# TianmingQiu/BNN_KFAC

Measured on AMD Instinct MI355X. Metric: images/sec for full KFAC factor pass + factor inversion, MNIST MLP, 1/2/4/8 GPUs, higher is better.
Workload: dtype f32; 1 GPU; C2: MLP 784-128-10 KFAC factor pass over 60000 images/rank (batch 4096/rank, global batch 4096) + invert(0.04000000000000001, 200); global_batch=4096, images_per_rank=60000, parallelism=dp1

## Files before the change

bnn_kfac_amd/_native.py:

```python
from __future__ import annotations

import atexit
import ctypes
import os
import threading

import torch

_HERE = os.path.dirname(os.path.abspath(__file__))
LIB_PATH = os.environ.get("BNN_KFAC_AMD_LIB", os.path.join(_HERE, "libkfac_hip.so"))

KFAC_OK, KFAC_EINVAL, KFAC_ELAUNCH, KFAC_EWORKSPACE = 0, -1, -2, -3
ROWMAJOR, CHANNEL, PATCH = 0, 1, 2
OUT_INV_CHOL, OUT_INVERSE = 0, 1
TRI_SYMMETRIC, TRI_LOWER = 0, 1
(PROF_FACTOR_TILES, PROF_FACTOR_REDUCE, PROF_INVERT, PROF_QUAD_TILES, PROF_FACTOR_SYRK3,
 PROF_FACTOR_X3, PROF_FACTOR_CONV, PROF_FACTOR_CHANNEL_SMALL, PROF_SYEV, PROF_FACTOR_CONV_X3,
 PROF_FACTOR_CONV_X3S, PROF_FACTOR_CONV_X3F, PROF_FACTOR_CHANNEL_X3) = range(13)
PROF_FACTOR_KERNELS = {PROF_FACTOR_TILES: "kfac_factor_tiles", PROF_FACTOR_SYRK3: "kfac_factor_syrk3",
                       PROF_FACTOR_X3: "kfac_factor_tiles_x3", PROF_FACTOR_CONV: "kfac_factor_conv",
                       PROF_FACTOR_CHANNEL_SMALL: "kfac_factor_channel_small",
                       PROF_FACTOR_CONV_X3: "kfac_factor_conv_x3", PROF_FACTOR_CONV_X3S: "kfac_factor_conv_x3s",
                       PROF_FACTOR_CONV_X3F: "kfac_factor_conv_x3f", PROF_FACTOR_CHANNEL_X3: "kfac_factor_channel_x3"}

# ... 83 lines not shown
                ("ld_diag", c_i64), ("nA", c_i32), ("nG", c_i32), ("accumulate", c_i32),
                ("scale", c_f32)]


class GramJob(ctypes.Structure):
    _fields_ = [("UA", c_vp), ("ldA", c_i64), ("UG", c_vp), ("ldG", c_i64), ("c", c_vp),
                ("sigma", c_vp), ("out", c_vp), ("ldo", c_i64), ("nA", c_i32), ("nG", c_i32),
                ("la", c_i32), ("lg", c_i32)]


class TriJob(ctypes.Structure):
    _fields_ = [("F", c_vp), ("ldF", c_i64), ("n", c_i32), ("reserved", c_i32), ("offset", c_i64)]


SIGNATURES = {
    "kfac_factor_workspace_bytes": (ctypes.c_size_t, [ctypes.POINTER(FactorJob), ctypes.c_int]),
    "kfac_factor_update": (ctypes.c_int, [ctypes.POINTER(FactorJob), ctypes.c_int, c_vp,
                                          ctypes.c_size_t, c_vp]),
    "kfac_factor_accum_plan": (ctypes.c_int, [ctypes.POINTER(FactorJob), ctypes.c_int,
                                              ctypes.POINTER(c_i32), ctypes.POINTER(ctypes.c_size_t)]),
    "kfac_factor_route": (ctypes.c_int, [ctypes.POINTER(FactorJob), ctypes.c_int, ctypes.POINTER(c_i32)]),
    "kfac_factor_flush": (ctypes.c_int, [ctypes.POINTER(FactorJob), ctypes.c_int, c_vp]),
    "kfac_x3_unit_table": (ctypes.c_int, [ctypes.c_int, ctypes.POINTER(c_i32), ctypes.c_int]),
    "kfac_syrk_linear": (ctypes.c_int, [c_vp, c_i64, c_i64, c_i64, ctypes.c_int, c_f32, c_f32,
                                        c_vp, c_i64, c_vp, ctypes.c_size_t, c_vp]),
    "kfac_syrk_conv": (ctypes.c_int, [c_vp, c_i64] + [ctypes.c_int] * 10 + [c_f32, c_f32, c_vp,
                                                                            c_i64, c_vp,
                                                                            ctypes.c_size_t, c_vp]),
    "kfac_syrk_convgrad": (ctypes.c_int, [c_vp, c_i64, ctypes.c_int, c_i64, c_f32, c_f32, c_vp,
                                          c_i64, c_vp, ctypes.c_size_t, c_vp]),
    "kfac_invert_workspace_bytes": (ctypes.c_size_t, [ctypes.POINTER(InvertJob), ctypes.c_int]),
    "kfac_invert": (ctypes.c_int, [ctypes.POINTER(InvertJob), ctypes.c_int, c_vp,
                                   ctypes.c_size_t, c_vp, c_vp]),
    "kfac_invert_ex": (ctypes.c_int, [ctypes.POINTER(InvertJob), ctypes.c_int, c_vp,
                                      ctypes.c_size_t, c_vp, c_vp, c_vp]),
    "kfac_damped_inv_chol": (ctypes.c_int, [c_vp, ctypes.c_int, c_i64, c_f64, c_f64, c_vp, c_i64,
                                            c_vp, ctypes.c_size_t, c_vp, c_vp]),
    "kfac_eig_workspace_bytes": (ctypes.c_size_t, [ctypes.POINTER(EigJob), ctypes.c_int]),
    "kfac_syev": (ctypes.c_int, [ctypes.POINTER(EigJob), ctypes.c_int, c_vp, ctypes.c_size_t,
                                 c_vp, c_vp]),
    "kfac_quadform_workspace_bytes": (ctypes.c_size_t, [ctypes.POINTER(QuadJob), ctypes.c_int,
                                                        c_i64]),
    "kfac_kron_quadform": (ctypes.c_int, [ctypes.POINTER(QuadJob), ctypes.c_int, c_i64,
                                          ctypes.c_int, c_vp, c_vp, ctypes.c_size_t, c_vp]),
    "kfac_kron_cov_workspace_bytes": (ctypes.c_size_t, [ctypes.POINTER(CovJob), ctypes.c_int, c_i64,
                                                        ctypes.c_int]),
# ... 663 lines not shown
```

bnn_kfac_amd/csrc/capi.hip:

```cpp
#include "kfac_common.h"

extern "C" const char* kfac_strerror(int status) {
  switch (status) {
    case KFAC_OK: return "ok";
    case KFAC_EINVAL: return "invalid argument";
    case KFAC_ELAUNCH: return "HIP kernel launch failed";
    case KFAC_EWORKSPACE: return "workspace too small";
    default: return "unknown kfac status";
  }
}

extern "C" const char* kfac_version(void) { return "bnn_kfac_amd 0.1.0 gfx950"; }

#include <stdlib.h>
#include <string.h>

#include <algorithm>
#include <atomic>

#include "knobs.h"

namespace kfac {
namespace {
int env_int(const char* name, int dflt) {
// ... 121 lines not shown
  int64_t cnt = 0;
  for (const Rec& r : g_done) {
    if (r.id != id) continue;
    if (hipEventSynchronize(r.stop) != hipSuccess) return KFAC_ELAUNCH;
    float ms = 0.f;
    if (hipEventElapsedTime(&ms, r.start, r.stop) != hipSuccess) return KFAC_ELAUNCH;
    tot += ms;
    wk += r.work;
    by += r.bytes;
    ++cnt;
  }
  if (total_ms) *total_ms = tot;
  if (launches) *launches = cnt;
  if (work) *work = wk;
  if (bytes) *bytes = by;
  return KFAC_OK;
}

extern "C" int kfac_profile_read(int id, double* total_ms, int64_t* launches) {
  return kfac_profile_read_work(id, total_ms, launches, nullptr, nullptr);
}

int kfac_release_graphs();

extern "C" int kfac_release(void) {
  int rc = kfac_release_graphs();
  std::lock_guard<std::mutex> lk(g_mu);
  g_on = false;
  for (const Rec& r : g_open) {
    (void)hipEventDestroy(r.start);
    (void)hipEventDestroy(r.stop);
  }
  for (const Rec& r : g_done) {
    if (hipEventSynchronize(r.stop) != hipSuccess) rc = KFAC_ELAUNCH;
    (void)hipEventDestroy(r.start);
    (void)hipEventDestroy(r.stop);
  }
  for (hipEvent_t e : g_pool) (void)hipEventDestroy(e);
  g_open.clear();
  g_done.clear();
  g_pool.clear();
  return rc;
}

extern "C" int kfac_event_create(void** ev) {
  if (!ev) return KFAC_EINVAL;
  return hipEventCreateWithFlags(reinterpret_cast<hipEvent_t*>(ev), hipEventDisableTiming) == hipSuccess
             ? KFAC_OK
             : KFAC_ELAUNCH;
// ... 35 lines not shown
```

bnn_kfac_amd/csrc/factor.hip:

```cpp
#include <algorithm>
#include <utility>
#include <vector>

#include "factor_common.h"

namespace kfac {

struct Plan {
  int tiles, splits;
  int units;
  int tasks;
  int64_t chunk;
  size_t slab_bytes;
};

static int factor_n(const kfac_factor_job& j) { return j.x.cols + (j.x.has_ones ? 1 : 0); }

static int64_t job_sps(const kfac_factor_job& j) { return std::max<int64_t>(1, cdiv(j.x.rows, BK)); }
static int job_nseg(const kfac_factor_job& j) { return j.nseg > 1 ? j.nseg : 1; }
static bool job_ragged(const kfac_factor_job& j) {
  return j.nseg > 1 && j.x.last_rows > 0 && j.x.last_rows < j.x.rows;
}
static int64_t job_stages(const kfac_factor_job& j) {
  if (job_ragged(j)) return job_sps(j) * (j.nseg - 1) + std::max<int64_t>(1, cdiv(j.x.last_rows, BK));
  return job_sps(j) * job_nseg(j);
}
static int64_t job_krows(const kfac_factor_job& j) {
  if (job_ragged(j)) return j.x.rows * (j.nseg - 1) + j.x.last_rows;
  return j.x.rows * job_nseg(j);
}
static double job_operand_bytes(const kfac_factor_job& j) {
  const double rows = (double)job_krows(j);
  if (j.x.layout == KFAC_PATCH)
    return rows / (double)std::max<int64_t>(1, j.x.L) * (double)j.x.C * j.x.H * j.x.W * sizeof(float);
  return rows * j.x.cols * sizeof(float);
}
// ... 97 lines not shown
    const uintptr_t* bases = reinterpret_cast<const uintptr_t*>(j.seg_ptrs);
    for (int64_t s = 0; s < nseg; ++s)
      if (bases[s] % 16 != 0) return false;
  }
  if (!conv_fp32_geom(o, g)) return false;
  r.family = o.layout != KFAC_CHANNEL ? KFAC_PROF_FACTOR_CONV
             : channel_small(g)       ? KFAC_PROF_FACTOR_CHANNEL_SMALL
             : channel_x3_geom(o, g)  ? KFAC_PROF_FACTOR_CHANNEL_X3 : KFAC_PROF_FACTOR_CONV;
  return true;
}

static Route route_group(const kfac_factor_job* jobs, int njobs) {
  Route r{};
  r.family = KFAC_PROF_FACTOR_TILES;
  if (syrk3_group(jobs, njobs))
    r.family = KFAC_PROF_FACTOR_SYRK3;
  else if (tiles_x3_group(jobs, njobs))
    r.family = KFAC_PROF_FACTOR_X3;
  else if (njobs == 1)
    conv_geom(jobs[0], r);
  return r;
}

static void plan_jobs(const kfac_factor_job* jobs, int njobs, const Route& route, Plan* plans) {
  const Family& fam = family_of(route);
  const bool s3 = route.family == KFAC_PROF_FACTOR_SYRK3, x3 = route.family == KFAC_PROF_FACTOR_X3;
  const int64_t slots = (int64_t)fam.wgs * 256;
  constexpr int64_t MIN_CHUNK = 8, OVERHEAD = 4;
  int64_t max_steps = 1;
  for (int i = 0; i < njobs; ++i) max_steps = std::max(max_steps, job_stages(jobs[i]));
  int64_t units[MAXJ];
  for (int i = 0; i < njobs; ++i) {
    const int n = factor_n(jobs[i]);
    const int64_t t = cdiv(n, TILE);
    units[i] = s3 ? syrk3_units(n) : x3 ? x3_units(n) : fam.images ? route.cg.units : t * (t + 1) / 2;
  }
  auto thin = [&](int i) {
    const int n = factor_n(jobs[i]);
    return x3 && n > TILE && (n - 1) % TILE < 32;
  };
  auto job_tasks = [&](int i, int64_t splits) { return units[i] * splits; };
  auto job_splits = [&](int i, int64_t c) { return cdiv(job_stages(jobs[i]), c); };
  auto tasks_at = [&](int64_t c) {
    int64_t n = 0;
    for (int i = 0; i < njobs; ++i)
      n += job_tasks(i, job_splits(i, c));
    return n;
  };
  int64_t best_c = std::max(MIN_CHUNK, max_steps), best_cost = -1;
  bool any_thin = false;
  for (int i = 0; i < njobs; ++i) any_thin |= thin(i);
  const int64_t max_rounds = any_thin ? 1 : (s3 ? 16 : 4);
  for (int64_t r = 1; r <= max_rounds; ++r) {
    int64_t lo = MIN_CHUNK, hi = std::max(MIN_CHUNK, max_steps);
    if (tasks_at(hi) > r * slots) continue;
    while (lo < hi) {
      const int64_t mid = (lo + hi) / 2;
      if (tasks_at(mid) <= r * slots) hi = mid; else lo = mid + 1;
    }
    const int64_t cost = (lo + OVERHEAD) * r;
    if (best_cost < 0 || cost < best_cost) { best_cost = cost; best_c = lo; }
  }
  for (int i = 0; i < njobs; ++i) {
    const int t = (int)cdiv(factor_n(jobs[i]), TILE);
    Plan& p = plans[i];
    p.tiles = t * (t + 1) / 2;
    p.units = (int)units[i];
    const int64_t steps = job_stages(jobs[i]);
    if (jobs[i].acc) {
      p.splits = jobs[i].acc_splits;
      p.chunk = cdiv(steps, (int64_t)p.splits);
      p.slab_bytes = 0;
      p.tasks = (int)job_tasks(i, p.splits);
      continue;
    }
    p.splits = (int)job_splits(i, best_c);
    if (fam.images) {
      const ConvGeom& cg = route.cg;
      const bool halve = route.family == KFAC_PROF_FACTOR_CHANNEL_SMALL && cg.B <= 8 * slots;
      int k = (int)std::max<int64_t>(1, cdiv((int64_t)cg.units * cg.B, halve ? slots / 2 : slots));
      if (knobs().conv_k > 0) k = knobs().conv_k;
      k = std::min(k, cg.B);
      p.splits = (int)cdiv(cg.B, k);
    }
    p.chunk = cdiv(steps, (int64_t)p.splits);
    p.slab_bytes = align_up((size_t)p.tiles * p.splits * TILE * TILE * sizeof(float), 256);
    p.tasks = (int)job_tasks(i, p.splits);
  }
}

static size_t accum_bytes(int n, int splits) {
// ... 34 lines not shown
  d.rdelta = 0;
  if (job_ragged(jb)) {
    d.rdelta = (int)(jb.x.rows - jb.x.last_rows);
    d.rstage = (int64_t)d.sps * (jb.nseg - 1);
    d.rw = (float)((double)jb.x.rows / (double)jb.x.last_rows);
    d.rinv = (float)((double)jb.x.last_rows / (double)jb.x.rows);
  }
}

struct GroupLaunch {
  FactorArgs args, red;
  int tasks, rtiles;
};

static int prepare_group(const kfac_factor_job* jobs, int njobs, const Route& route, char* ws,
                         size_t ws_bytes, GroupLaunch& g) {
  Plan plans[MAXJ];
  plan_jobs(jobs, njobs, route, plans);
  FactorArgs& args = g.args;
  FactorArgs& red = g.red;
  args = FactorArgs{};
  red = FactorArgs{};
  args.njobs = njobs;
  args.split_major = 1;
  int tasks = 0, rtiles = 0, nsegs = 0;
  size_t off = 0;
  for (int i = 0; i < njobs; ++i) {
    const kfac_factor_job& jb = jobs[i];
    FactorJobDev& d = args.job[i];
    fill_dev(d, jb);
    d.glds = job_glds(jb);
    d.x3units = route.family == KFAC_PROF_FACTOR_X3 ? plans[i].units : 0;
    d.splits = plans[i].splits;
    d.sstride = jb.acc && jb.acc_stride > 0 ? jb.acc_stride : d.splits;
    d.chunk = plans[i].chunk;
    if (d.nseg > 1) {
      const float* const* bases = reinterpret_cast<const float* const*>(jb.seg_ptrs);
      d.seg_off = nsegs;
      for (int s = 0; s < d.nseg; ++s) args.segs[nsegs++] = bases[s];
    }
    if (jb.acc) {
      d.slab = jb.acc;
    } else {
      d.slab = reinterpret_cast<float*>(ws + off);
      off += plans[i].slab_bytes;
      FactorJobDev& e = red.job[red.njobs];
      e = d;
      e.tile_begin = rtiles;
      rtiles += plans[i].tiles;
      red.tile_end[red.njobs++] = rtiles;
    }
    d.task_begin = tasks;
    tasks += plans[i].tasks;
    args.task_end[i] = tasks;
  }
  g.tasks = tasks;
  g.rtiles = rtiles;
  return off > ws_bytes ? KFAC_EWORKSPACE : KFAC_OK;
}

static int factor_group(const kfac_factor_job* jobs, int njobs, const Route& route, char* ws,
                        size_t ws_bytes, hipStream_t stream) {
  GroupLaunch g;
  const int rc = prepare_group(jobs, njobs, route, ws, ws_bytes, g);
  if (rc != KFAC_OK) return rc;
  if (g.tasks == 0) return KFAC_OK;
  {
    double work = 0.0, bytes = 0.0;
    if (prof_on())
      for (int i = 0; i < njobs; ++i) {
// ... 65 lines not shown
    if (j.acc && (j.acc_splits <= 0 || j.acc_splits > (1 << 20))) return KFAC_EINVAL;
    if (j.acc && j.acc_stride != 0 && (j.acc_stride < j.acc_splits || j.acc_stride > (1 << 20)))
      return KFAC_EINVAL;
    if (j.nseg < 0 || (j.nseg > 1 && !j.seg_ptrs) || job_sps(j) > (1 << 30))
      return KFAC_EINVAL;
    if (j.x.last_rows < 0 || j.x.last_rows > j.x.rows ||
        (job_ragged(j) && j.x.layout != KFAC_ROWMAJOR))
      return KFAC_EINVAL;
  }
  return KFAC_OK;
}

extern "C" int kfac_factor_accum_plan(const kfac_factor_job* jobs, int njobs, int32_t* splits,
                                      size_t* bytes) {
  if (validate(jobs, njobs) != KFAC_OK || (njobs > 0 && (!splits || !bytes))) return KFAC_EINVAL;
  std::vector<kfac_factor_job> sorted;
  std::vector<int> order;
  std::vector<std::pair<int, int>> groups;
  launch_groups(jobs, njobs, sorted, order, groups);
  for (auto& j : sorted) j.acc = nullptr;
  for (const auto& g : groups) {
    Plan plans[MAXJ];
    const kfac_factor_job* gj = sorted.data() + g.first;
    plan_jobs(gj, g.second, route_group(gj, g.second), plans);
    for (int k = 0; k < g.second; ++k) {
      const int i = order[g.first + k];
      splits[i] = plans[k].splits;
      bytes[i] = accum_bytes(factor_n(jobs[i]), plans[k].splits);
    }
  }
  return KFAC_OK;
}

extern "C" int kfac_factor_route(const kfac_factor_job* jobs, int njobs, int32_t* family) {
  if (validate(jobs, njobs) != KFAC_OK || (njobs > 0 && !family)) return KFAC_EINVAL;
  std::vector<kfac_factor_job> sorted;
  std::vector<int> order;
  std::vector<std::pair<int, int>> groups;
  launch_groups(jobs, njobs, sorted, order, groups);
  for (const auto& g : groups) {
    const int fam = route_group(sorted.data() + g.first, g.second).family;
    for (int k = 0; k < g.second; ++k) family[order[g.first + k]] = fam;
  }
  return KFAC_OK;
}

static int update_group(const kfac_factor_job* gj, int n, void* workspace, size_t workspace_bytes,
// ... 189 lines not shown
```

bnn_kfac_amd/csrc/factor_common.h:

```cpp
#pragma once

#include <cstddef>

#include "kfac_common.h"

namespace kfac {

constexpr int MAXJ = 16;
constexpr int KSEG = 64;

struct FactorJobDev {
  OpDev x;
  float alpha, beta;
  float* F;
  int64_t ldF;
  float* slab;
  int seg_off;
  int64_t chunk;
  int64_t nst;
  int sps, nseg;
  int n, t, splits;
  int task_begin;
  int glds;
  int tile_begin;
  int accum;
// ... 54 lines not shown
    if (i >= nb) break;
#pragma unroll
    for (int v = 0; v < 16; ++v) *at(i, v) = upd ? fmaf(J.sbeta, old[i][v], a * acc[i][v]) : a * acc[i][v];
  }
}

__device__ __forceinline__ const float* seg_base(const FactorJobDev& J, const float* const* segs,
                                                 int seg) {
  return J.seg_off >= 0 ? segs[J.seg_off + seg] : J.x.ptr;
}

__device__ __forceinline__ int64_t seg_rows(const FactorJobDev& J, int seg) {
  return J.x.rows - (int64_t)(seg == J.nseg - 1) * J.rdelta;
}

template <int NA>
__device__ __forceinline__ void scale_acc(floatx16 (&acc)[NA], float f) {
#pragma unroll
  for (int a = 0; a < NA; ++a)
#pragma unroll
    for (int v = 0; v < 16; ++v) acc[a][v] *= f;
}

struct StageCursor {
  int seg;
  int64_t k;
  __device__ __forceinline__ void init(const FactorJobDev& J, int64_t s) {
    seg = (int)(s / J.sps);
    k = (s - (int64_t)seg * J.sps) * BK;
  }
  __device__ __forceinline__ void next(int64_t rows) {
    k += BK;
    if (k >= rows) { k = 0; ++seg; }
  }
};

template <int NW = 4>
__device__ __forceinline__ void store_narrow(const FactorJobDev& J, float* out, floatx16& acc,
                                             float* lds) {
  const int lane = threadIdx.x & 63, wave = threadIdx.x >> 6;
  __syncthreads();
  if (wave > 0) {
#pragma unroll
    for (int v = 0; v < 16; ++v) lds[((wave - 1) * 16 + v) * 64 + lane] = acc[v];
  }
  __syncthreads();
  if (wave != 0) return;
#pragma unroll
  for (int w = 0; w < NW - 1; ++w)
#pragma unroll
    for (int v = 0; v < 16; ++v) acc[v] += lds[(w * 16 + v) * 64 + lane];
  put_partial(J, acc, [&](int v) { return &out[acc_row(v, lane) * TILE + (lane & 31)]; });
}

template <int NW = 4>
__device__ __forceinline__ void narrow_direct_load(const FactorJobDev& J, const float* base, int64_t k0,
                                                   int64_t rows, float (&v)[BK / (2 * NW)]) {
  const int lane = threadIdx.x & 63, wave = threadIdx.x >> 6, rr = lane & 31, h = lane >> 5;
#pragma unroll
  for (int s2 = 0; s2 < BK / (2 * NW); ++s2) {
    const int64_t k = k0 + 2 * (wave * (BK / (2 * NW)) + s2) + h;
    v[s2] = k < rows ? (rr < J.x.cols ? base[k * J.x.ld + rr] : (rr == J.x.ones ? 1.f : 0.f)) : 0.f;
  }
}

template <int NW = 4>
__device__ __forceinline__ void factor_task_narrow_direct(const FactorJobDev& J, const float* const* segs,
                                                          int local, float* lds) {
  constexpr int NV = BK / (2 * NW);
  const int split = local;
  const int64_t s0 = (int64_t)split * J.chunk;
  const int64_t s1 = min(J.nst, s0 + J.chunk);
  floatx16 acc[1];
#pragma unroll
  for (int v = 0; v < 16; ++v) acc[0][v] = 0.f;
  if (s1 > s0) {
    StageCursor c;
    c.init(J, s0);
    const float* base = seg_base(J, segs, c.seg);
    float cur[NV], nxt[NV];
    narrow_direct_load<NW>(J, base, c.k, seg_rows(J, c.seg), cur);
    for (int64_t s = s0; s < s1; ++s) {
      const int seg = c.seg;
      c.next(J.x.rows);
      if (s + 1 < s1) {
        if (c.seg != seg) base = seg_base(J, segs, c.seg);
        narrow_direct_load<NW>(J, base, c.k, seg_rows(J, c.seg), nxt);
      }
      if (s == J.rstage && s > s0) scale_acc(acc, J.rinv);
#pragma unroll
      for (int s2 = 0; s2 < NV; ++s2)
        acc[0] = __builtin_amdgcn_mfma_f32_32x32x2f32(cur[s2], cur[s2], acc[0], 0, 0, 0);
#pragma unroll
      for (int s2 = 0; s2 < NV; ++s2) cur[s2] = nxt[s2];
    }
    if (J.rstage >= 0 && s1 > J.rstage) scale_acc(acc, J.rw);
  }
  store_narrow<NW>(J, J.slab + (size_t)split * TILE * TILE, acc[0], lds);
}

constexpr int CONV_SRC_MAX = 2048;

typedef float floatx4 __attribute__((ext_vector_type(4)));

enum ConvMode {
  CONV_BLOCKS = 0,
  CONV_N16 = 2,
  CONV_N32 = 3,
};

struct ConvGeom {
  int mode;
  int n;
  int KR;
  int B;
  int bseg;
  int T;
  int G;
  int stride;
  int rowstep;
  int Ho;
// ... 28 lines not shown
  int xf_one, xf_zero, xf_dummy;
  int xf_nks;
  int xf_wave[4];
  int xs_lb[32];
  int8_t xs_f[32];
  int xf_cb[128];
};


static inline int raise_dynamic_lds(const void* kernel, int bytes) {
  return hipFuncSetAttribute(kernel, hipFuncAttributeMaxDynamicSharedMemorySize, bytes) == hipSuccess
             ? KFAC_OK : KFAC_ELAUNCH;
}

constexpr int TILES_WGS = 4;
int launch_tiles(const FactorArgs& args, int tasks, hipStream_t stream);
void launch_reduce(const FactorArgs& red, int tiles, hipStream_t stream);

constexpr int S3D_WGS = 2;
int64_t syrk3_units(int n);
int launch_syrk3(const FactorArgs& args, int tasks, hipStream_t stream);

constexpr int X3_WGS = 4;
constexpr int X3_PMAX = 64;
constexpr int X3_UCAP = 2048;
constexpr uint32_t X3_DIAG = 1u << 28;
struct X3Units {
  uint32_t u[X3_UCAP];
};
__host__ __device__ inline int x3_unit_np(uint32_t u) { return (int)(u >> 24) & 7; }
__host__ __device__ inline int x3_unit_panel(uint32_t u, int s) { return (int)(u >> (6 * s)) & 63; }
static inline int x3_panels(int n) { return (n + 31) / 32; }
int x3_unit_table(int P, const uint32_t** table);
int x3_units(int n);
int x3_table_entries(const int* n, int njobs);
int launch_tiles_x3(const FactorArgs& args, int tasks, hipStream_t stream);

constexpr int KFAC_CONV_OCC = 4;
bool conv_fp32_geom(const kfac_operand& o, ConvGeom& g);
int launch_conv(const FactorArgs& args, const ConvGeom& g, int tasks, hipStream_t stream);

constexpr int CONV_X3_WGS = 1;
bool conv_x3_geom(const kfac_operand& o, ConvGeom& g);
int launch_conv_x3(const FactorArgs& args, const ConvGeom& g, int tasks, hipStream_t stream);
bool conv_x3s_geom(const kfac_operand& o, ConvGeom& g);
int launch_conv_x3s(const FactorArgs& args, const ConvGeom& g, int tasks, hipStream_t stream);
bool conv_x3f_geom(const kfac_operand& o, ConvGeom& g);
int launch_conv_x3f(const FactorArgs& args, const ConvGeom& g, int tasks, hipStream_t stream);

constexpr int CHANNEL_WGS = 4;
bool channel_small(const ConvGeom& g);
bool channel_x3_geom(const kfac_operand& o, ConvGeom& g);
int launch_channel_x3(const FactorArgs& args, const ConvGeom& g, int tasks, hipStream_t stream);
int launch_channel_small(const FactorArgs& args, const ConvGeom& g, int tasks, hipStream_t stream);

}
```

bnn_kfac_amd/csrc/factor_tiles_x3.hip:

```cpp
#include <algorithm>
#include <mutex>
#include <type_traits>
#include <vector>

#include "bf16x3.h"
#include "factor_common.h"

namespace kfac {

constexpr int X3_THREADS = 128;

constexpr int X3_NW = X3_THREADS / 64;

struct X3Col {
  int voff;
  bool fill;
  float fv;
};

__device__ __forceinline__ void x3_load8(float (&x)[8], __amdgpu_buffer_rsrc_t rs, const X3Col& c,
                                         int sbase, int sstep) {
#pragma unroll
  for (int r = 0; r < 8; ++r)
    x[r] = __uint_as_float(__builtin_amdgcn_raw_buffer_load_b32(rs, c.voff, sbase + r * sstep, 0));
// ... 140 lines not shown
      x3_pattern<NV>();
      __builtin_amdgcn_sched_barrier(0);
      F1n = take(1, kn, kns, c2);
      x3_six(acc[2], F2, F1);
      x3_pattern<NV>();
    } else {
      F0n = take(0, kn, kns, c2);
      F1n = take(1, kn, kns, c2);
      x3_six(acc[0], F1, F0);
      x3_pattern<2 * NV>();
    }
    kc = kn;
    kcs = kns;
  };
  const int64_t rst = J.rstage;
  const int bst = (rst > s0 && rst < s1) ? (int)(rst - s0) : -1;
  for (int st = 0; st < ns; ++st) {
    if (st == bst) scale_acc(acc, J.rinv);
    X3Frag qa, qb;
    stage(pa, pb, qa, qb);
    pa = qa;
    pb = qb;
  }
  if (rst >= 0 && s1 > rst) scale_acc(acc, J.rw);
}

template <int KIND>
__device__ __forceinline__ void x3_unit(const FactorJobDev& J, const float* const* segs, const int (&pn)[4],
                                        int np, int split, float* lds) {
  constexpr bool DIAG = KIND == X3_KDIAG;
  constexpr int NB = x3_kind_blocks(KIND);
  const int64_t s0 = (int64_t)split * J.chunk;
  const int64_t s1 = min(J.nst, s0 + J.chunk);
  const int lane = threadIdx.x & 63;
  const int wave = __builtin_amdgcn_readfirstlane(threadIdx.x >> 6);
  floatx16 acc[NB];
#pragma unroll
  for (int b = 0; b < NB; ++b)
#pragma unroll
    for (int v = 0; v < 16; ++v) acc[b][v] = 0.f;
  if (s1 > s0) {
    const int op = J.x.ones >> 5;
    const bool fill = J.x.ones >= 0 && (pn[0] == op || pn[1] == op || pn[2] == op || pn[3] == op);
    if (fill) x3_loop<KIND, true>(J, segs, pn, s0, s1, acc);
    else x3_loop<KIND, false>(J, segs, pn, s0, s1, acc);
  }
  const int nblk = DIAG ? np : NB;
  constexpr int HALF = (NB + 1) / 2;
  __syncthreads();
#pragma unroll
  for (int b = 0; b < NB; ++b) {
    const bool mine = (b < HALF) == (wave == 0);
    if (b < nblk && !mine)
#pragma unroll
      for (int v = 0; v < 16; ++v) lds[(b * 16 + v) * 64 + lane] = acc[b][v];
  }
  __syncthreads();
#pragma unroll
  for (int b = 0; b < NB; ++b) {
    const bool mine = (b < HALF) == (wave == 0);
    if (b >= nblk || !mine) continue;
    constexpr int BI[6] = {1, 2, 2, 3, 3, 3}, BJ[6] = {0, 0, 1, 0, 1, 2};
    const int pr = DIAG ? pn[b & 3] : pn[BI[b]], pc = DIAG ? pn[b & 3] : pn[BJ[b]];
    const int ti = pr >> 1, tj = pc >> 1;
    float* out = J.slab + ((size_t)(ti * (ti + 1) / 2 + tj) * J.sstride + split) * TILE * TILE +
                 (pr & 1) * 32 * TILE + (pc & 1) * 32;
#pragma unroll
    for (int v = 0; v < 16; ++v) acc[b][v] += lds[(b * 16 + v) * 64 + lane];
    put_partial(J, acc[b], [&](int v) { return &out[acc_row(v, lane) * TILE + (lane & 31)]; });
  }
}

template <int GBK>
__device__ __forceinline__ void factor_task_x3(const FactorJobDev& J, const float* const* segs,
                                               const X3Units& U, int local, float* lds, int split_major) {
  static_assert(GBK == 16 * X3_NW, "one 16-row half stage per wave");
  const int units = J.x3units;
  const int split = split_major ? local / units : local % J.splits;
  const int unit = split_major ? local - split * units : local / J.splits;
  const uint32_t u = U.u[J.x3tab + unit];
  const int np = x3_unit_np(u);
  const int pn[4] = {x3_unit_panel(u, 0), x3_unit_panel(u, 1), x3_unit_panel(u, 2), x3_unit_panel(u, 3)};
  switch ((u & X3_DIAG) ? X3_KDIAG : np) {
    case 4: x3_unit<4>(J, segs, pn, np, split, lds); break;
    case 3: x3_unit<3>(J, segs, pn, np, split, lds); break;
    case 2: x3_unit<2>(J, segs, pn, np, split, lds); break;
    case X3_KDIAG: x3_unit<X3_KDIAG>(J, segs, pn, np, split, lds); break;
    default: break;
  }
}

__global__ __launch_bounds__(X3_THREADS, 2) void kfac_factor_tiles_x3(FactorArgs args, X3Units units) {
  __shared__ __attribute__((aligned(16))) float lds[X3_NACC * 16 * 64];
  const int task = xcd_task(blockIdx.x, gridDim.x);
  int j = 0;
  while (j + 1 < args.njobs && task >= args.task_end[j]) ++j;
  const int local = task - args.job[j].task_begin;
  const FactorJobDev& J = args.job[j];
  if (J.n <= 32)
    factor_task_narrow_direct<X3_NW>(J, args.segs, local, lds);
  else
    factor_task_x3<BK>(J, args.segs, units, local, lds, args.split_major);
}

namespace {

uint32_t x3_pack(const int* p, int np, bool diag) {
  uint32_t u = (uint32_t)np << 24 | (diag ? X3_DIAG : 0u);
  for (int s = 0; s < 4; ++s) u |= (uint32_t)p[std::min(s, np - 1)] << (6 * s);
  return u;
}

std::vector<uint32_t> x3_build_table(int P) {
  std::vector<uint32_t> k4, k3, k2, dg;
  std::vector<char> used((size_t)P * P, 0);
  auto is_free = [&](int a, int b) { return !used[(size_t)a * P + b]; };
  auto mark = [&](int a, int b) { used[(size_t)a * P + b] = used[(size_t)b * P + a] = 1; };
  if (P == 25) {
    const int base[4][2] = {{0, 0}, {0, 1}, {1, 0}, {2, 2}};
    for (int m = 1; m <= 2; ++m)
      for (int sx = 0; sx < 5; ++sx)
        for (int sy = 0; sy < 5; ++sy) {
          int p[4];
          for (int i = 0; i < 4; ++i) p[i] = 5 * ((m * base[i][0] + sx) % 5) + (m * base[i][1] + sy) % 5;
          std::sort(p, p + 4);
// ... 50 lines not shown
  static std::mutex mu;
  static std::vector<uint32_t> tables[X3_PMAX + 1];
  if (P < 2 || P > X3_PMAX) return 0;
  std::lock_guard<std::mutex> lock(mu);
  if (tables[P].empty()) tables[P] = x3_build_table(P);
  if (table) *table = tables[P].data();
  return (int)tables[P].size();
}

int x3_units(int n) { return n <= 32 ? 1 : x3_unit_table(x3_panels(n), nullptr); }

int x3_table_entries(const int* n, int njobs) {
  bool seen[X3_PMAX + 1] = {};
  int total = 0;
  for (int i = 0; i < njobs; ++i) {
    const int P = x3_panels(n[i]);
    if (n[i] <= 32 || P > X3_PMAX || seen[P]) continue;
    seen[P] = true;
    total += x3_unit_table(P, nullptr);
  }
  return total;
}

int launch_tiles_x3(const FactorArgs& args, int tasks, hipStream_t stream) {
  FactorArgs a = args;
  X3Units U;
  int off[X3_PMAX + 1], total = 0;
  std::fill(off, off + X3_PMAX + 1, -1);
  for (int i = 0; i < a.njobs; ++i) {
    FactorJobDev& d = a.job[i];
    d.x3tab = 0;
    if (d.n <= 32) continue;
    const int P = x3_panels(d.n);
    const uint32_t* t = nullptr;
    const int nu = x3_unit_table(P, &t);
    if (nu == 0 || nu != d.x3units) return KFAC_ELAUNCH;
    if (off[P] < 0) {
      if (total + nu > X3_UCAP) return KFAC_ELAUNCH;
      std::copy(t, t + nu, U.u + total);
      off[P] = total;
      total += nu;
    }
    d.x3tab = off[P];
  }
  std::fill(U.u + total, U.u + X3_UCAP, 0u);
  hipLaunchKernelGGL(kfac_factor_tiles_x3, dim3(tasks), dim3(X3_THREADS), 0, stream, a, U);
  return KFAC_OK;
}

}

extern "C" int kfac_x3_unit_table(int P, int32_t* out, int cap) {
  const uint32_t* t = nullptr;
  const int nu = kfac::x3_unit_table(P, &t);
  for (int i = 0; i < nu && i < cap && out; ++i) {
    const int np = kfac::x3_unit_np(t[i]);
    const bool diag = (t[i] & kfac::X3_DIAG) != 0;
    for (int s = 0; s < 4; ++s) out[6 * i + s] = s < np ? kfac::x3_unit_panel(t[i], s) : -1;
    out[6 * i + 4] = diag ? 0 : (np == 4 ? 63 : np == 3 ? 0b001011 : 0b000001);
    out[6 * i + 5] = diag ? (1 << np) - 1 : 0;
  }
  return nu;
}
```

include/kfac_hip.h:

```cpp
#ifndef KFAC_HIP_H
#define KFAC_HIP_H

#include <stddef.h>
#include <stdint.h>

#ifdef __cplusplus
extern "C" {
#endif

#if defined(__GNUC__) || defined(__clang__)
#define KFAC_API __attribute__((visibility("default")))
#else
#define KFAC_API
#endif

typedef void* kfac_stream_t;

enum kfac_status {
  KFAC_OK = 0,
  KFAC_EINVAL = -1,
  KFAC_ELAUNCH = -2,
  KFAC_EWORKSPACE = -3,
};

// ... 16 lines not shown
  kfac_operand x;
  float alpha;
  float beta;
  float* F;
  int64_t ldF;
  float* acc;
  int32_t acc_splits;
  float acc_beta;
  const void* seg_ptrs;
  int32_t nseg;
  int32_t acc_stride;
} kfac_factor_job;

KFAC_API size_t kfac_factor_workspace_bytes(const kfac_factor_job* jobs, int njobs);
KFAC_API int kfac_factor_update(const kfac_factor_job* jobs, int njobs, void* workspace,
                       size_t workspace_bytes, kfac_stream_t stream);

KFAC_API int kfac_factor_accum_plan(const kfac_factor_job* jobs, int njobs, int32_t* splits,
                           size_t* bytes);
KFAC_API int kfac_factor_route(const kfac_factor_job* jobs, int njobs, int32_t* family);
KFAC_API int kfac_factor_flush(const kfac_factor_job* jobs, int njobs, kfac_stream_t stream);

KFAC_API int kfac_x3_unit_table(int P, int32_t* out, int cap);

KFAC_API int kfac_syrk_linear(const float* x, int64_t B, int64_t d, int64_t ldx, int has_ones,
                     float alpha, float beta, float* F, int64_t ldF, void* workspace,
                     size_t workspace_bytes, kfac_stream_t stream);
KFAC_API int kfac_syrk_conv(const float* x, int64_t B, int C, int H, int W, int kh, int kw, int sh,
                   int sw, int ph, int pw, int has_ones, float alpha, float beta, float* F,
                   int64_t ldF, void* workspace, size_t workspace_bytes, kfac_stream_t stream);
KFAC_API int kfac_syrk_convgrad(const float* g, int64_t B, int C, int64_t L, float alpha, float beta,
                       float* F, int64_t ldF, void* workspace, size_t workspace_bytes,
                       kfac_stream_t stream);

enum kfac_inv_out { KFAC_OUT_INV_CHOL = 0, KFAC_OUT_INVERSE = 1 };

typedef struct kfac_invert_job {
  const float* F;
  int64_t ldF;
  int32_t n;
  int32_t out_kind;
  double scale;
  double shift;
  float* out;
  int64_t ldo;
} kfac_invert_job;
// ... 296 lines not shown
```

Measured before the change: 214.3 million images/s.

## Cost-balanced ragged stage-range work split for x3 factor kernel

Adds a host-side planner that cuts the combined (unit, stage) work of all factor jobs into roughly equal-cost pieces per workgroup. Each workgroup handles up to three ranged pieces, and the schedule is arranged per XCD. It also zeroes unused split slabs and fixes the ragged-stage scaling for partial ranges. The aim is to remove load imbalance and tail waste from fixed split×unit task grids. The cost is a cached device table, more launch-path logic, and more reduction slabs.

```diff
diff --git a/bnn_kfac_amd/_native.py b/bnn_kfac_amd/_native.py
--- a/bnn_kfac_amd/_native.py
+++ b/bnn_kfac_amd/_native.py
@@ -129,6 +129,8 @@
     "kfac_factor_route": (ctypes.c_int, [ctypes.POINTER(FactorJob), ctypes.c_int, ctypes.POINTER(c_i32)]),
     "kfac_factor_flush": (ctypes.c_int, [ctypes.POINTER(FactorJob), ctypes.c_int, c_vp]),
     "kfac_x3_unit_table": (ctypes.c_int, [ctypes.c_int, ctypes.POINTER(c_i32), ctypes.c_int]),
+    "kfac_x3_task_ranges": (ctypes.c_int, [ctypes.POINTER(ctypes.c_int), ctypes.POINTER(c_i64), ctypes.c_int,
+                                           ctypes.c_int, ctypes.POINTER(c_i32), ctypes.c_int]),
     "kfac_syrk_linear": (ctypes.c_int, [c_vp, c_i64, c_i64, c_i64, ctypes.c_int, c_f32, c_f32,
                                         c_vp, c_i64, c_vp, ctypes.c_size_t, c_vp]),
     "kfac_syrk_conv": (ctypes.c_int, [c_vp, c_i64] + [ctypes.c_int] * 10 + [c_f32, c_f32, c_vp,
diff --git a/bnn_kfac_amd/csrc/capi.hip b/bnn_kfac_amd/csrc/capi.hip
--- a/bnn_kfac_amd/csrc/capi.hip
+++ b/bnn_kfac_amd/csrc/capi.hip
@@ -167,9 +167,11 @@
 }
 
 int kfac_release_graphs();
+namespace kfac { void x3_release(); }
 
 extern "C" int kfac_release(void) {
   int rc = kfac_release_graphs();
+  kfac::x3_release();
   std::lock_guard<std::mutex> lk(g_mu);
   g_on = false;
   for (const Rec& r : g_open) {
diff --git a/bnn_kfac_amd/csrc/factor.hip b/bnn_kfac_amd/csrc/factor.hip
--- a/bnn_kfac_amd/csrc/factor.hip
+++ b/bnn_kfac_amd/csrc/factor.hip
@@ -12,6 +12,7 @@
   int tasks;
   int64_t chunk;
   size_t slab_bytes;
+  bool ranges;
 };
 
 static int factor_n(const kfac_factor_job& j) { return j.x.cols + (j.x.has_ones ? 1 : 0); }
@@ -155,7 +156,8 @@
   return r;
 }
 
-static void plan_jobs(const kfac_factor_job* jobs, int njobs, const Route& route, Plan* plans) {
+static void plan_jobs(const kfac_factor_job* jobs, int njobs, const Route& route, Plan* plans,
+                      bool layout = false) {
   const Family& fam = family_of(route);
   const bool s3 = route.family == KFAC_PROF_FACTOR_SYRK3, x3 = route.family == KFAC_PROF_FACTOR_X3;
   const int64_t slots = (int64_t)fam.wgs * 256;
@@ -194,12 +196,30 @@
     const int64_t cost = (lo + OVERHEAD) * r;
     if (best_cost < 0 || cost < best_cost) { best_cost = cost; best_c = lo; }
   }
+  const X3Cut* cut = nullptr;
+  if (x3) {
+    int n[MAXJ];
+    int64_t st[MAXJ];
+    for (int i = 0; i < njobs; ++i) n[i] = factor_n(jobs[i]), st[i] = job_stages(jobs[i]);
+    cut = x3_cut(n, st, njobs, (int)slots);
+    if (layout && cut && !cut->full) cut = nullptr;
+    for (int i = 0; cut && i < njobs; ++i)
+      if (jobs[i].acc && jobs[i].acc_splits < cut->need[i]) cut = nullptr;
+  }
   for (int i = 0; i < njobs; ++i) {
     const int t = (int)cdiv(factor_n(jobs[i]), TILE);
     Plan& p = plans[i];
     p.tiles = t * (t + 1) / 2;
     p.units = (int)units[i];
+    p.ranges = cut != nullptr;
     const int64_t steps = job_stages(jobs[i]);
+    if (cut) {
+      p.splits = jobs[i].acc ? jobs[i].acc_splits : cut->need[i];
+      p.chunk = steps;
+      p.slab_bytes = jobs[i].acc ? 0 : align_up((size_t)p.tiles * p.splits * TILE * TILE * sizeof(float), 256);
+      p.tasks = i == 0 ? cut->grid : 0;
+      continue;
+    }
     if (jobs[i].acc) {
       p.splits = jobs[i].acc_splits;
       p.chunk = cdiv(steps, (int64_t)p.splits);
@@ -280,7 +300,7 @@
   args = FactorArgs{};
   red = FactorArgs{};
   args.njobs = njobs;
-  args.split_major = 1;
+  args.split_major = njobs > 0 && plans[0].ranges ? 2 : 1;
   int tasks = 0, rtiles = 0, nsegs = 0;
   size_t off = 0;
   for (int i = 0; i < njobs; ++i) {
@@ -304,6 +324,7 @@
       off += plans[i].slab_bytes;
       FactorJobDev& e = red.job[red.njobs];
       e = d;
+      if (d.rstage >= 0) e.alpha = d.alpha * d.rw;
       e.tile_begin = rtiles;
       rtiles += plans[i].tiles;
       red.tile_end[red.njobs++] = rtiles;
@@ -415,7 +436,7 @@
   for (const auto& g : groups) {
     Plan plans[MAXJ];
     const kfac_factor_job* gj = sorted.data() + g.first;
-    plan_jobs(gj, g.second, route_group(gj, g.second), plans);
+    plan_jobs(gj, g.second, route_group(gj, g.second), plans, true);
     for (int k = 0; k < g.second; ++k) {
       const int i = order[g.first + k];
       splits[i] = plans[k].splits;
diff --git a/bnn_kfac_amd/csrc/factor_common.h b/bnn_kfac_amd/csrc/factor_common.h
--- a/bnn_kfac_amd/csrc/factor_common.h
+++ b/bnn_kfac_amd/csrc/factor_common.h
@@ -1,6 +1,7 @@
 #pragma once
 
 #include <cstddef>
+#include <vector>
 
 #include "kfac_common.h"
 
@@ -101,6 +102,17 @@
     for (int v = 0; v < 16; ++v) acc[a][v] *= f;
 }
 
+template <int NA>
+__device__ __forceinline__ void ragged_finish(const FactorJobDev& J, floatx16 (&acc)[NA], int64_t s1) {
+  if (J.rstage < 0) return;
+  const bool reached = s1 > J.rstage;
+  if (J.accum) {
+    if (reached) scale_acc(acc, J.rw);
+  } else if (!reached) {
+    scale_acc(acc, J.rinv);
+  }
+}
+
 struct StageCursor {
   int seg;
   int64_t k;
@@ -145,11 +157,8 @@
 
 template <int NW = 4>
 __device__ __forceinline__ void factor_task_narrow_direct(const FactorJobDev& J, const float* const* segs,
-                                                          int local, float* lds) {
+                                                          int64_t s0, int64_t s1, int split, float* lds) {
   constexpr int NV = BK / (2 * NW);
-  const int split = local;
-  const int64_t s0 = (int64_t)split * J.chunk;
-  const int64_t s1 = min(J.nst, s0 + J.chunk);
   floatx16 acc[1];
 #pragma unroll
   for (int v = 0; v < 16; ++v) acc[0][v] = 0.f;
@@ -173,9 +182,16 @@
 #pragma unroll
       for (int s2 = 0; s2 < NV; ++s2) cur[s2] = nxt[s2];
     }
-    if (J.rstage >= 0 && s1 > J.rstage) scale_acc(acc, J.rw);
+    ragged_finish(J, acc, s1);
   }
   store_narrow<NW>(J, J.slab + (size_t)split * TILE * TILE, acc[0], lds);
+}
+
+template <int NW = 4>
+__device__ __forceinline__ void factor_task_narrow_direct(const FactorJobDev& J, const float* const* segs,
+                                                          int local, float* lds) {
+  const int64_t s0 = (int64_t)local * J.chunk;
+  factor_task_narrow_direct<NW>(J, segs, s0, min(J.nst, s0 + J.chunk), local, lds);
 }
 
 constexpr int CONV_SRC_MAX = 2048;
@@ -250,12 +266,22 @@
 int launch_syrk3(const FactorArgs& args, int tasks, hipStream_t stream);
 
 constexpr int X3_WGS = 4;
+constexpr int X3_SLOTS = 256 * X3_WGS;
 constexpr int X3_PMAX = 64;
-constexpr int X3_UCAP = 2048;
+constexpr int X3_UCAP = 2046;
 constexpr uint32_t X3_DIAG = 1u << 28;
+struct X3Piece {
+  int64_t s0, s1;
+  uint32_t ju;
+  int32_t slab;
+};
+constexpr int X3_RP = 3;
+constexpr uint32_t X3_LAST = 1u << 31;
 struct X3Units {
+  const X3Piece* ranges;
   uint32_t u[X3_UCAP];
 };
+static_assert(sizeof(X3Units) == 8192, "the unit tables and the range table's address: 8 KB of kernel arguments");
 __host__ __device__ inline int x3_unit_np(uint32_t u) { return (int)(u >> 24) & 7; }
 __host__ __device__ inline int x3_unit_panel(uint32_t u, int s) { return (int)(u >> (6 * s)) & 63; }
 static inline int x3_panels(int n) { return (n + 31) / 32; }
@@ -263,6 +289,18 @@
 int x3_units(int n);
 int x3_table_entries(const int* n, int njobs);
 int launch_tiles_x3(const FactorArgs& args, int tasks, hipStream_t stream);
+struct X3Cut {
+  int W;
+  int grid;
+  std::vector<X3Piece> lin;
+  std::vector<X3Piece> disp;
+  int need[MAXJ];
+  int64_t cost_min, cost_max;
+  bool full;
+  const X3Piece* dev[16];
+};
+const X3Cut* x3_cut(const int* n, const int64_t* stages, int njobs, int slots);
+void x3_release();
 
 constexpr int KFAC_CONV_OCC = 4;
 bool conv_fp32_geom(const kfac_operand& o, ConvGeom& g);
diff --git a/bnn_kfac_amd/csrc/factor_tiles_x3.hip b/bnn_kfac_amd/csrc/factor_tiles_x3.hip
--- a/bnn_kfac_amd/csrc/factor_tiles_x3.hip
+++ b/bnn_kfac_amd/csrc/factor_tiles_x3.hip
@@ -186,16 +186,14 @@
     pa = qa;
     pb = qb;
   }
-  if (rst >= 0 && s1 > rst) scale_acc(acc, J.rw);
+  ragged_finish(J, acc, s1);
 }
 
 template <int KIND>
 __device__ __forceinline__ void x3_unit(const FactorJobDev& J, const float* const* segs, const int (&pn)[4],
-                                        int np, int split, float* lds) {
+                                        int np, int64_t s0, int64_t s1, int split, int clear, float* lds) {
   constexpr bool DIAG = KIND == X3_KDIAG;
   constexpr int NB = x3_kind_blocks(KIND);
-  const int64_t s0 = (int64_t)split * J.chunk;
-  const int64_t s1 = min(J.nst, s0 + J.chunk);
   const int lane = threadIdx.x & 63;
   const int wave = __builtin_amdgcn_readfirstlane(threadIdx.x >> 6);
   floatx16 acc[NB];
@@ -232,39 +230,80 @@
 #pragma unroll
     for (int v = 0; v < 16; ++v) acc[b][v] += lds[(b * 16 + v) * 64 + lane];
     put_partial(J, acc[b], [&](int v) { return &out[acc_row(v, lane) * TILE + (lane & 31)]; });
+    if (clear > split + 1) {
+#pragma unroll
+      for (int v = 0; v < 16; ++v) acc[b][v] = 0.f;
+      for (int s = split + 1; s < clear; ++s) {
+        float* z = out + (size_t)(s - split) * TILE * TILE;
+        put_partial(J, acc[b], [&](int v) { return &z[acc_row(v, lane) * TILE + (lane & 31)]; });
+      }
+    }
   }
 }
 
 template <int GBK>
 __device__ __forceinline__ void factor_task_x3(const FactorJobDev& J, const float* const* segs,
-                                               const X3Units& U, int local, float* lds, int split_major) {
+                                               const X3Units& U, int unit, int64_t s0, int64_t s1, int split,
+                                               int clear, float* lds) {
   static_assert(GBK == 16 * X3_NW, "one 16-row half stage per wave");
-  const int units = J.x3units;
-  const int split = split_major ? local / units : local % J.splits;
-  const int unit = split_major ? local - split * units : local / J.splits;
   const uint32_t u = U.u[J.x3tab + unit];
   const int np = x3_unit_np(u);
   const int pn[4] = {x3_unit_panel(u, 0), x3_unit_panel(u, 1), x3_unit_panel(u, 2), x3_unit_panel(u, 3)};
   switch ((u & X3_DIAG) ? X3_KDIAG : np) {
-    case 4: x3_unit<4>(J, segs, pn, np, split, lds); break;
-    case 3: x3_unit<3>(J, segs, pn, np, split, lds); break;
-    case 2: x3_unit<2>(J, segs, pn, np, split, lds); break;
-    case X3_KDIAG: x3_unit<X3_KDIAG>(J, segs, pn, np, split, lds); break;
+    case 4: x3_unit<4>(J, segs, pn, np, s0, s1, split, clear, lds); break;
+    case 3: x3_unit<3>(J, segs, pn, np, s0, s1, split, clear, lds); break;
+    case 2: x3_unit<2>(J, segs, pn, np, s0, s1, split, clear, lds); break;
+    case X3_KDIAG: x3_unit<X3_KDIAG>(J, segs, pn, np, s0, s1, split, clear, lds); break;
     default: break;
+  }
+}
+
+__device__ __forceinline__ void x3_piece(const FactorJobDev& J, const float* const* segs, const X3Units& U,
+                                         int unit, int64_t s0, int64_t s1, int split, int clear, float* lds) {
+  if (J.n <= 32) {
+    factor_task_narrow_direct<X3_NW>(J, segs, s0, s1, split, lds);
+    if (clear > split + 1 && threadIdx.x < 64) {
+      const int lane = threadIdx.x;
+      floatx16 z;
+#pragma unroll
+      for (int v = 0; v < 16; ++v) z[v] = 0.f;
+      for (int s = split + 1; s < clear; ++s) {
+        float* out = J.slab + (size_t)s * TILE * TILE;
+        put_partial(J, z, [&](int v) { return &out[acc_row(v, lane) * TILE + (lane & 31)]; });
+      }
+    }
+  } else {
+    factor_task_x3<BK>(J, segs, U, unit, s0, s1, split, clear, lds);
   }
 }
 
 __global__ __launch_bounds__(X3_THREADS, 2) void kfac_factor_tiles_x3(FactorArgs args, X3Units units) {
   __shared__ __attribute__((aligned(16))) float lds[X3_NACC * 16 * 64];
-  const int task = xcd_task(blockIdx.x, gridDim.x);
-  int j = 0;
-  while (j + 1 < args.njobs && task >= args.task_end[j]) ++j;
-  const int local = task - args.job[j].task_begin;
-  const FactorJobDev& J = args.job[j];
-  if (J.n <= 32)
-    factor_task_narrow_direct<X3_NW>(J, args.segs, local, lds);
-  else
-    factor_task_x3<BK>(J, args.segs, units, local, lds, args.split_major);
+  static_assert(sizeof(X3Piece) == 24, "six words per piece");
+  uint32_t w[6];
+  if (units.ranges) {
+    const uint32_t* r = reinterpret_cast<const uint32_t*>(units.ranges + blockIdx.x);
+#pragma unroll
+    for (int i = 0; i < 6; ++i) w[i] = __builtin_amdgcn_readfirstlane(r[i]);
+    if (w[0] == w[2] && w[1] == w[3]) return;
+  } else {
+    const int task = xcd_task(blockIdx.x, gridDim.x);
+    int j = 0;
+    while (j + 1 < args.njobs && task >= args.task_end[j]) ++j;
+    const int local = task - args.job[j].task_begin;
+    const FactorJobDev& J = args.job[j];
+    const int units_j = J.n <= 32 ? 1 : J.x3units;
+    const int split = local / units_j;
+    const int64_t s0 = (int64_t)split * J.chunk, s1 = min(J.nst, s0 + J.chunk);
+    w[0] = (uint32_t)s0, w[1] = (uint32_t)((uint64_t)s0 >> 32);
+    w[2] = (uint32_t)s1, w[3] = (uint32_t)((uint64_t)s1 >> 32);
+    w[4] = (uint32_t)(local - split * units_j) | (uint32_t)j << 16;
+    w[5] = (uint32_t)split;
+  }
+  const int64_t s0 = (int64_t)((uint64_t)w[0] | (uint64_t)w[1] << 32);
+  const int64_t s1 = (int64_t)((uint64_t)w[2] | (uint64_t)w[3] << 32);
+  const FactorJobDev& J = args.job[(w[4] >> 16) & 0xff];
+  x3_piece(J, args.segs, units, (int)(w[4] & 0xffff), s0, s1, (int)w[5], (w[4] & X3_LAST) ? J.splits : 0, lds);
 }
 
 namespace {
@@ -361,9 +400,214 @@
   return total;
 }
 
+namespace {
+
+struct CutUnit {
+  int job, unit, cost;
+  int64_t stages, begin;
+};
+
+int x3_unit_cost(uint32_t u) {
+  const int np = x3_unit_np(u);
+  return (u & X3_DIAG) ? 6 * np : 6 * (np * (np - 1) / 2);
+}
+constexpr int X3_COST_NARROW = 16;
+constexpr int X3_COST_MAX = 36;
+constexpr int64_t X3_MIN_STAGES = 8;
+
+bool x3_cut_at(const std::vector<CutUnit>& U, int64_t total, int64_t W, X3Cut& c) {
+  c.lin.clear();
+  std::fill(c.need, c.need + MAXJ, 0);
+  c.cost_min = total;
+  c.cost_max = 0;
+  std::vector<int> pieces(U.size(), 0);
+  const int64_t lo = total / W / X3_COST_MAX * X3_COST_MAX, hi = lo + X3_COST_MAX;
+  size_t k = 0;
+  int64_t j = 0, at = 0;
+  for (int64_t w = 1; w <= W; ++w) {
+    size_t k1 = U.size();
+    int64_t j1 = 0, end = total;
+    if (w < W && at + lo < total) {
+      const int64_t T = (int64_t)((unsigned __int128)w * (unsigned __int128)total / (unsigned __int128)W);
+      size_t q = k;
+      while (q + 1 < U.size() && U[q + 1].begin <= at + lo) ++q;
+      int64_t best = -1;
+      for (; q < U.size() && U[q].begin <= at + hi; ++q) {
+        const int64_t b = U[q].begin, cq = U[q].cost;
+        const int64_t jlo = std::max<int64_t>(0, (at + lo - b + cq - 1) / cq);
+        const int64_t jhi = std::min<int64_t>(U[q].stages, (at + hi - b) / cq);
+        if (jlo > jhi) continue;
+        const int64_t jn = std::min(jhi, std::max(jlo, T > b ? (T - b + (cq - 1) / 2) / cq : 0));
+        const int64_t pos = b + jn * cq;
+        if (pos <= at) continue;
+        if (best < 0 || std::llabs(pos - T) < std::llabs(best - T)) {
+          best = pos;
+          k1 = q;
+          j1 = jn;
+        }
+      }
+      if (best >= 0) {
+        end = best;
+        if (j1 >= U[k1].stages) ++k1, j1 = 0;
+      } else {
+        k1 = U.size(), j1 = 0;
+      }
+    }
+    if (end <= at) continue;
+    int np = 0;
+    X3Piece p[X3_RP];
+    for (size_t q = k; q < U.size() && (q < k1 || (q == k1 && j1 > 0)); ++q) {
+      const int64_t s0 = q == k ? j : 0, s1 = q == k1 ? j1 : U[q].stages;
+      if (np == X3_RP) return false;
+      const bool last = s1 == U[q].stages;
+      p[np].s0 = s0;
+      p[np].s1 = s1;
+      p[np].ju = (uint32_t)U[q].unit | (uint32_t)U[q].job << 16 | (last ? X3_LAST : 0u);
+      p[np].slab = pieces[q]++;
+      ++np;
+    }
+    for (int i = np; i < X3_RP; ++i) p[i] = X3Piece{0, 0, 0u, 0};
+    c.lin.insert(c.lin.end(), p, p + X3_RP);
+    c.cost_min = std::min(c.cost_min, end - at);
+    c.cost_max = std::max(c.cost_max, end - at);
+    k = k1;
+    j = j1;
+    at = end;
+  }
+  for (size_t q = 0; q < U.size(); ++q) c.need[U[q].job] = std::max(c.need[U[q].job], pieces[q]);
+  c.W = (int)(c.lin.size() / X3_RP);
+  return true;
+}
+
+bool x3_cut_search(const std::vector<CutUnit>& U, int64_t total, int slots, X3Cut& c) {
+  int64_t W = std::max<int64_t>(1, std::min<int64_t>(slots, total / (X3_MIN_STAGES * X3_COST_MAX)));
+  for (; W <= (1 << 20); W += std::max<int64_t>(1, W / 8))
+    if (x3_cut_at(U, total, W, c)) return true;
+  return false;
+}
+
+std::mutex g_cut_mu;
+std::vector<std::pair<std::vector<int64_t>, X3Cut*>> g_cuts;
+
+}
+
+const X3Cut* x3_cut(const int* n, const int64_t* stages, int njobs, int slots) {
+  if (njobs <= 0 || njobs > MAXJ || slots <= 0) return nullptr;
+  std::vector<int64_t> key;
+  key.reserve(2 * njobs + 1);
+  key.push_back(slots);
+  for (int i = 0; i < njobs; ++i) key.push_back(n[i]), key.push_back(stages[i]);
+  std::lock_guard<std::mutex> lock(g_cut_mu);
+  for (const auto& e : g_cuts)
+    if (e.first == key) return e.second;
+  std::vector<CutUnit> U;
+  int64_t total = 0;
+  for (int i = 0; i < njobs; ++i) {
+    if (n[i] <= 0 || stages[i] <= 0 || stages[i] > ((int64_t)1 << 40)) return nullptr;
+    const uint32_t* t = nullptr;
+    const int nu = n[i] <= 32 ? 1 : x3_unit_table(x3_panels(n[i]), &t);
+    if (nu <= 0 || nu > 0xffff) return nullptr;
+    for (int u = 0; u < nu; ++u) {
+      const int cost = n[i] <= 32 ? X3_COST_NARROW : x3_unit_cost(t[u]);
+      U.push_back(CutUnit{i, u, cost, stages[i], total});
+      total += cost * stages[i];
+    }
+  }
+  X3Cut* c = new X3Cut();
+  std::fill(c->dev, c->dev + 16, nullptr);
+  const bool ok = x3_cut_search(U, total, slots, *c);
+  c->full = total >= (int64_t)slots * X3_MIN_STAGES * X3_COST_MAX;
+  if (!ok) {
+    delete c;
+    c = nullptr;
+  } else {
+    std::vector<int> order(c->W);
+    for (int r = 0; r < c->W; ++r) order[r] = r;
+    std::stable_sort(order.begin(), order.end(), [&](int a, int b) {
+      const X3Piece &pa = c->lin[(size_t)a * X3_RP], &pb = c->lin[(size_t)b * X3_RP];
+      const uint32_t ja = (pa.ju >> 16) & 0xff, jb = (pb.ju >> 16) & 0xff;
+      if (ja != jb) return ja < jb;
+      if (pa.s0 != pb.s0) return pa.s0 < pb.s0;
+      return (pa.ju & 0xffff) < (pb.ju & 0xffff);
+    });
+    auto piece_cost = [&](const X3Piece& q) {
+      const int job = (int)((q.ju >> 16) & 0xff);
+      int cost = X3_COST_NARROW;
+      if (n[job] > 32) {
+        const uint32_t* t = nullptr;
+        x3_unit_table(x3_panels(n[job]), &t);
+        cost = x3_unit_cost(t[q.ju & 0xffff]);
+      }
+      return (q.s1 - q.s0) * cost;
+    };
+    const int W = c->W, per = W >> 3, rem = W & 7, base = (W + 7) & ~7;
+    std::vector<X3Piece> later[8];
+    c->disp.assign(base, X3Piece{0, 0, 0u, 0});
+    for (int b = 0; b < W; ++b) {
+      const int x = b & 7;
+      const int task = (x < rem ? x * (per + 1) : rem * (per + 1) + (x - rem) * per) + (b >> 3);
+      const X3Piece* q = &c->lin[(size_t)order[task] * X3_RP];
+      c->disp[b] = q[0];
+      for (int i = 1; i < X3_RP; ++i)
+        if (q[i].s1 > q[i].s0) later[x].push_back(q[i]);
+    }
+    size_t deep = 0;
+    for (int x = 0; x < 8; ++x) {
+      std::stable_sort(later[x].begin(), later[x].end(),
+                       [&](const X3Piece& a, const X3Piece& b) { return piece_cost(a) > piece_cost(b); });
+      deep = std::max(deep, later[x].size());
+    }
+    c->disp.resize(base + 8 * deep, X3Piece{0, 0, 0u, 0});
+    for (int x = 0; x < 8; ++x)
+      for (size_t i = 0; i < later[x].size(); ++i) c->disp[base + 8 * i + x] = later[x][i];
+    c->grid = (int)c->disp.size();
+  }
+  g_cuts.emplace_back(std::move(key), c);
+  return c;
+}
+
+static const X3Piece* x3_cut_device(const X3Cut* cut) {
+  int dev = 0;
+  if (hipGetDevice(&dev) != hipSuccess || dev < 0 || dev >= 16) return nullptr;
+  std::lock_guard<std::mutex> lock(g_cut_mu);
+  X3Cut* c = const_cast<X3Cut*>(cut);
+  if (!c->dev[dev]) {
+    const std::vector<X3Piece>& t = c->disp;
+    void* p = nullptr;
+    if (hipMalloc(&p, t.size() * sizeof(X3Piece)) != hipSuccess) return nullptr;
+    if (hipMemcpy(p, t.data(), t.size() * sizeof(X3Piece), hipMemcpyHostToDevice) != hipSuccess) {
+      (void)hipFree(p);
+      return nullptr;
+    }
+    c->dev[dev] = static_cast<const X3Piece*>(p);
+  }
+  return c->dev[dev];
+}
+
+void x3_release() {
+  std::lock_guard<std::mutex> lock(g_cut_mu);
+  for (auto& e : g_cuts)
+    if (e.second)
+      for (int d = 0; d < 16; ++d) {
+        if (e.second->dev[d]) (void)hipFree(const_cast<X3Piece*>(e.second->dev[d]));
+        e.second->dev[d] = nullptr;
+      }
+}
+
 int launch_tiles_x3(const FactorArgs& args, int tasks, hipStream_t stream) {
   FactorArgs a = args;
   X3Units U;
+  U.ranges = nullptr;
+  if (a.split_major == 2) {
+    int n[MAXJ];
+    int64_t st[MAXJ];
+    for (int i = 0; i < a.njobs; ++i) n[i] = a.job[i].n, st[i] = a.job[i].nst;
+    const X3Cut* cut = x3_cut(n, st, a.njobs, X3_SLOTS);
+    if (!cut || cut->grid != tasks) return KFAC_ELAUNCH;
+    for (int i = 0; i < a.njobs; ++i)
+      if (a.job[i].splits < cut->need[i]) return KFAC_ELAUNCH;
+    if (!(U.ranges = x3_cut_device(cut))) return KFAC_ELAUNCH;
+  }
   int off[X3_PMAX + 1], total = 0;
   std::fill(off, off + X3_PMAX + 1, -1);
   for (int i = 0; i < a.njobs; ++i) {
@@ -401,3 +645,28 @@
   }
   return nu;
 }
+
+extern "C" int kfac_x3_task_ranges(const int* n, const int64_t* stages, int njobs, int slots, int32_t* out,
+                                   int cap) {
+  if (!n || !stages || njobs <= 0 || njobs > kfac::MAXJ || slots <= 0) return 0;
+  for (int i = 0; i < njobs; ++i)
+    if (n[i] <= 0 || kfac::x3_panels(n[i]) > kfac::X3_PMAX || stages[i] <= 0 || stages[i] > INT32_MAX) return 0;
+  const kfac::X3Cut* c = kfac::x3_cut(n, stages, njobs, slots);
+  if (!c) return 0;
+  for (int r = 0; r < c->W && r < cap && out; ++r) {
+    int np = 0;
+    for (int p = 0; p < kfac::X3_RP; ++p) {
+      const kfac::X3Piece& q = c->lin[(size_t)r * kfac::X3_RP + p];
+      const bool live = q.s1 > q.s0;
+      np += live;
+      int32_t* o = out + 16 * r + 5 * p;
+      o[0] = live ? (int32_t)((q.ju >> 16) & 0xff) : -1;
+      o[1] = live ? (int32_t)(q.ju & 0xffff) : -1;
+      o[2] = (int32_t)q.s0;
+      o[3] = (int32_t)q.s1;
+      o[4] = live ? q.slab : -1;
+    }
+    out[16 * r + 15] = np;
+  }
+  return c->W;
+}
diff --git a/include/kfac_hip.h b/include/kfac_hip.h
--- a/include/kfac_hip.h
+++ b/include/kfac_hip.h
@@ -62,6 +62,8 @@
 KFAC_API int kfac_factor_flush(const kfac_factor_job* jobs, int njobs, kfac_stream_t stream);
 
 KFAC_API int kfac_x3_unit_table(int P, int32_t* out, int cap);
+KFAC_API int kfac_x3_task_ranges(const int* n, const int64_t* stages, int njobs, int slots,
+                                 int32_t* out, int cap);
 
 KFAC_API int kfac_syrk_linear(const float* x, int64_t B, int64_t d, int64_t ldx, int has_ones,
                      float alpha, float beta, float* F, int64_t ldF, void* workspace,
```

After: 62.33 million images/s. 70.9% lower.
